# rotationalio/honu

Measured on AMD Instinct MI355X. Metric: GiB/s + records/s device-resident encode+decode, 1M Large(~300KB) object batch, higher is better.
Workload: dtype u8

## Files before the change

### honu_amd/csrc/lane.h

```cpp
#pragma once

#include "common.h"

namespace honu {

HONU_DEV void window16(const u32x4 a, const u32x4 b, uint32_t s, uint64_t &lo, uint64_t &hi) {
    const uint32_t q4 = s >> 2, sh = s & 3;
    const uint32_t w0 = a.x, w1 = a.y, w2 = a.z, w3 = a.w, w4 = b.x, w5 = b.y, w6 = b.z, w7 = b.w;
    const bool o1 = q4 & 1, o2 = q4 & 2;
#define PICK(j0, j1, j2, j3) (o2 ? (o1 ? (j3) : (j2)) : (o1 ? (j1) : (j0)))
    const uint32_t p0 = PICK(w0, w1, w2, w3);
    const uint32_t p1 = PICK(w1, w2, w3, w4);
    const uint32_t p2 = PICK(w2, w3, w4, w5);
    const uint32_t p3 = PICK(w3, w4, w5, w6);
    const uint32_t p4 = PICK(w4, w5, w6, w7);
#undef PICK
    const uint32_t r0 = __builtin_amdgcn_alignbyte(p1, p0, sh);
    const uint32_t r1 = __builtin_amdgcn_alignbyte(p2, p1, sh);
    const uint32_t r2 = __builtin_amdgcn_alignbyte(p3, p2, sh);
    const uint32_t r3 = __builtin_amdgcn_alignbyte(p4, p3, sh);
    lo = ((uint64_t)r1 << 32) | r0;
    hi = ((uint64_t)r3 << 32) | r2;
}

HONU_DEV void lane_fetch16(const uint8_t *__restrict__ base, uint64_t q, uint64_t end,
                           uint64_t &lo, uint64_t &hi) {
    const uint64_t A = q & ~15ull;
    const uint32_t s = (uint32_t)(q & 15);
    const u32x4 a = *reinterpret_cast<const u32x4 *>(base + A);
    u32x4 b = {0, 0, 0, 0};
    if (s && A + 16 < end) b = *reinterpret_cast<const u32x4 *>(base + A + 16);
    window16(a, b, s, lo, hi);
}

HONU_DEV uint64_t compact7(uint64_t x) {
    x = (x & 0x007F007F007F007Full) | ((x & 0x7F007F007F007F00ull) >> 1);
    x = (x & 0x00003FFF00003FFFull) | ((x & 0x3FFF00003FFF0000ull) >> 2);
    x = (x & 0x000000000FFFFFFFull) | ((x & 0x0FFFFFFF00000000ull) >> 4);
    return x;
}

HONU_DEV uint32_t uvarint_window(uint64_t lo, uint64_t hi, uint32_t n, uint64_t &v) {
    const uint64_t tl = ~lo & 0x8080808080808080ull;
    const uint64_t th = ~hi & 0x0000000000008080ull;
    uint32_t k;
    if (tl) k = (uint32_t)(__builtin_ctzll(tl) >> 3) + 1;
    else if (th) k = (uint32_t)(__builtin_ctzll(th) >> 3) + 9;
    else k = 11;
    if (k > n) return 0;
    if (k == 10 && ((hi >> 8) & 0xFF) > 1) return 0;
    const uint64_t m = k >= 8 ? lo : (lo & ((1ull << (8 * k)) - 1));
    uint64_t x = compact7(m & 0x7F7F7F7F7F7F7F7Full);
    if (k >= 9) x |= (hi & 0x7F) << 56;
    if (k == 10) x |= ((hi >> 8) & 0x7F) << 63;
    v = x;
    return k;
}

template <int NDW> struct RowT {
    uint32_t d[NDW];
    HONU_DEV void clear() {
#pragma unroll
        for (int i = 0; i < NDW; i++) d[i] = 0;
    }
    HONU_DEV void u8(int off, uint32_t v) { d[off >> 2] |= (v & 0xFF) << (8 * (off & 3)); }
    HONU_DEV void u32(int off, uint32_t v) { d[off >> 2] = v; }
    HONU_DEV void u64(int off, uint64_t v) {
        d[off >> 2] = (uint32_t)v;
        d[(off >> 2) + 1] = (uint32_t)(v >> 32);
    }
    HONU_DEV void bytes16(int off, uint64_t lo, uint64_t hi) {
        u64(off, lo);
        u64(off + 8, hi);
    }
    HONU_DEV void span(int off, uint64_t o, uint64_t l) {
        u64(off, o);
        u64(off + 8, l);
    }
    template <class T> HONU_DEV void store(T *dst) const {
        static_assert(sizeof(T) == 4 * NDW, "row size");
        u32x4 *p = reinterpret_cast<u32x4 *>(dst);
#pragma unroll
        for (int i = 0; i < NDW / 4; i++)
            p[i] = u32x4{d[4 * i], d[4 * i + 1], d[4 * i + 2], d[4 * i + 3]};
    }
};
using Row = RowT<88>;

struct GlobalSrc {
    const uint8_t *base;
    HONU_DEV uint32_t u8(uint64_t p) const { return base[p]; }
    HONU_DEV void fetch16(uint64_t p, uint64_t end, uint64_t &lo, uint64_t &hi) const {
        lane_fetch16(base, p, end, lo, hi);
    }
};

template <class Src> struct DecT {
    Src src;
    uint64_t p, end, tstart;

    HONU_DEV int u8(uint32_t &v) {
        if (p >= end) return HONU_ERR_EOF;
        v = src.u8(p);
        p += 1;
        return HONU_OK;
    }
    HONU_DEV int boolean(uint32_t &v) {
        int st = u8(v);
        if (st) return st;
        return v > 1 ? HONU_ERR_PARSE_BOOLEAN : HONU_OK;
    }
    HONU_DEV int uv(uint32_t maxw, int err, uint64_t &v) {
        if (p >= end) return HONU_ERR_EOF;
        const uint64_t avail = end - p;
        const uint32_t n = avail < maxw ? (uint32_t)avail : maxw;
        uint64_t lo, hi;
        src.fetch16(p, end, lo, hi);
        const uint32_t k = uvarint_window(lo, hi, n, v);
        if (!k) return err;
        p += k;
        return HONU_OK;
    }
    HONU_DEV int u32(uint32_t &v) {
        uint64_t x = 0;
        int st = uv(5, HONU_ERR_PARSE_VARINT, x);
        v = (uint32_t)x;
        return st;
    }
    HONU_DEV int u64(uint64_t &v) { return uv(10, HONU_ERR_PARSE_VARINT, v); }
    HONU_DEV int i64(int64_t &v) {
        uint64_t x = 0;
        int st = uv(10, HONU_ERR_PARSE_VARINT, x);
        v = unzigzag(x);
        return st;
    }
    HONU_DEV int ulid(uint64_t &lo, uint64_t &hi) {
        if (p >= end) return HONU_ERR_EOF;
        if (p + 16 > end) return HONU_ERR_UNEXPECTED_EOF;
        src.fetch16(p, end, lo, hi);
        p += 16;
        return HONU_OK;
    }
    HONU_DEV int frame(uint64_t &off, uint64_t &len) {
        uint64_t rl = 0;
        int st = uv(10, HONU_ERR_NO_LENGTH, rl);
        if (st) return st;
        if (rl >= (1ull << 63)) return HONU_ERR_PANIC;
        if (rl == 0) {
            off = 0;
            len = 0;
            return HONU_OK;
        }
        if (rl > (uint64_t)INT64_MAX - (p - tstart)) return HONU_ERR_PANIC;
        if (p + rl > end) return HONU_ERR_UNEXPECTED_EOF;
        off = p;
        len = rl;
        p += rl;
        return HONU_OK;
    }
};
using LaneDec = DecT<GlobalSrc>;

HONU_DEV uint32_t uvarint_bytes(uint64_t x, uint64_t &lo, uint64_t &hi) {
    const uint32_t n = uvarint_len(x);
    uint64_t y = x & 0x00FFFFFFFFFFFFFFull;
    y = (y & 0x000000000FFFFFFFull) | ((y & 0x00FFFFFFF0000000ull) << 4);
    y = (y & 0x00003FFF00003FFFull) | ((y & 0x0FFFC0000FFFC000ull) << 2);
    y = (y & 0x007F007F007F007Full) | ((y & 0x3F803F803F803F80ull) << 1);
    const uint32_t nl = n < 8 ? n : 8;
    const uint64_t cont = n > 8 ? 0x8080808080808080ull
                                : (0x8080808080808080ull & ((1ull << (8 * (nl - 1))) - 1));
    lo = (y | cont) & (nl == 8 ? ~0ull : ((1ull << (8 * nl)) - 1));
    hi = 0;
    if (n > 8) hi = ((x >> 56) & 0x7F) | (n > 9 ? 0x80 : 0) | ((x >> 63) << 8);
    return n;
}

template <int R>
struct LaneWriterT {
    uint8_t *out;
    uint64_t cpos;
    uint32_t f;
    uint32_t first;
    uint64_t a0, a1;
    uint64_t hpos;
    uint32_t hfirst;
    uint64_t h0, h1;
    u32x4 *ring;
    uint32_t nch;

    HONU_DEV void init(uint8_t *o, uint64_t pos) {
        out = o;
        cpos = pos & ~15ull;
        f = first = (uint32_t)(pos & 15);
        a0 = a1 = 0;
        hfirst = 0;
        nch = 0;
    }
    HONU_DEV void set_ring(u32x4 *r) { ring = r; }
    static HONU_DEV void store_bytes(uint8_t *p, uint32_t from, uint32_t to, uint64_t b0, uint64_t b1) {
        uint32_t j = from;
        auto bytes_at = [&](uint32_t k, uint32_t n) -> uint64_t {
            uint64_t v = k < 8 ? (b0 >> (8 * k)) | (k ? b1 << (64 - 8 * k) : 0) : b1 >> (8 * (k - 8));
            return n == 8 ? v : v & ((1ull << (8 * n)) - 1);
        };
        if ((j & 1) && j < to) { p[j] = (uint8_t)bytes_at(j, 1); j += 1; }
        if ((j & 2) && j + 2 <= to) { *reinterpret_cast<uint16_t *>(p + j) = (uint16_t)bytes_at(j, 2); j += 2; }
        if ((j & 4) && j + 4 <= to) { *reinterpret_cast<uint32_t *>(p + j) = (uint32_t)bytes_at(j, 4); j += 4; }
        if (j + 8 <= to) { *reinterpret_cast<uint64_t *>(p + j) = bytes_at(j, 8); j += 8; }
        if (j + 4 <= to) { *reinterpret_cast<uint32_t *>(p + j) = (uint32_t)bytes_at(j, 4); j += 4; }
        if (j + 2 <= to) { *reinterpret_cast<uint16_t *>(p + j) = (uint16_t)bytes_at(j, 2); j += 2; }
        if (j < to) p[j] = (uint8_t)bytes_at(j, 1);
    }
    HONU_DEV void flush() {
        if (first == 0) {
            const u32x4 v{(uint32_t)a0, (uint32_t)(a0 >> 32), (uint32_t)a1, (uint32_t)(a1 >> 32)};
            if constexpr (R > 0) {
                ring[((cpos >> 4) & (R - 1)) * HONU_WAVE] = v;
                nch++;
            } else {
                *reinterpret_cast<u32x4 *>(out + cpos) = v;
            }
        } else {
            hpos = cpos;
            hfirst = first;
            h0 = a0;
            h1 = a1;
            first = 0;
        }
        cpos += 16;
    }
    HONU_DEV void put(uint64_t v, uint32_t n) {
        const uint32_t s = 8 * f;
        uint64_t t2 = 0;
        if (s < 64) {
            a0 |= v << s;
            if (s) a1 |= v >> (64 - s);
        } else {
            a1 |= v << (s - 64);
            if (s > 64) t2 = v >> (128 - s);
        }
        f += n;
        if (f >= 16) {
            flush();
            a0 = t2;
            a1 = 0;
            f -= 16;
        }
    }
    HONU_DEV void byte(uint32_t v) { put(v & 0xFF, 1); }
    HONU_DEV void put16(uint64_t lo, uint64_t hi) {
        put(lo, 8);
        put(hi, 8);
    }
    HONU_DEV void uv(uint64_t x) {
        uint64_t lo, hi;
        const uint32_t n = uvarint_bytes(x, lo, hi);
        put(lo, n < 8 ? n : 8);
        if (n > 8) put(hi, n - 8);
    }
    HONU_DEV void run(const uint8_t *src, uint64_t len) {
        const uint64_t a = (uint64_t)src & 15;
        const u32x4 *w = reinterpret_cast<const u32x4 *>(src - a);
        const uint64_t nw = (a + len + 15) >> 4;
        const uint32_t sh = (uint32_t)(a & 7) * 8, hw = (uint32_t)(a >> 3);
        for (uint64_t k = 0; k < len; k += 64) {
            drain();
            const uint64_t q0 = (a + k) >> 4;
            uint64_t x[11];
#pragma unroll
            for (int j = 0; j < 5; j++) {
                u32x4 v{0, 0, 0, 0};
                if (q0 + j < nw) v = w[q0 + j];
                x[2 * j] = ((uint64_t)v.y << 32) | v.x;
                x[2 * j + 1] = ((uint64_t)v.w << 32) | v.z;
            }
            x[10] = 0;
#pragma unroll
            for (int j = 0; j < 8; j++) {
                const uint64_t off = k + 8 * j;
                if (off < len) {
                    const uint64_t take = len - off < 8 ? len - off : 8;
                    const uint64_t lo = hw ? x[j + 1] : x[j], hi = hw ? x[j + 2] : x[j + 1];
                    uint64_t v = sh ? (lo >> sh) | (hi << (64 - sh)) : lo;
                    if (take < 8) v &= (1ull << (8 * take)) - 1;
                    put(v, (uint32_t)take);
                }
            }
        }
    }
    HONU_DEV void frame(const uint8_t *var, honu_span sp) {
        uv(sp.len);
        run(var + sp.off, sp.len);
    }
    HONU_DEV void drain_all() {
        if constexpr (R > 0) {
            const uint64_t p0 = cpos - 16ull * nch;
            for (uint32_t k = 0; k < nch; k++)
                *reinterpret_cast<u32x4 *>(out + p0 + 16 * k) = ring[(((p0 >> 4) + k) & (R - 1)) * HONU_WAVE];
            nch = 0;
        }
    }
    HONU_DEV void drain() {
        if constexpr (R == 16) {
            const uint64_t p0 = cpos - 16ull * nch, lim = cpos & ~127ull;
            if (p0 < lim) {
                const uint32_t cnt = (uint32_t)((lim - p0) >> 4);
                for (uint32_t k = 0; k < cnt; k++)
                    *reinterpret_cast<u32x4 *>(out + p0 + 16 * k) = ring[(((p0 >> 4) + k) & (R - 1)) * HONU_WAVE];
                nch -= cnt;
            }
        } else {
            drain_all();
        }
    }
    HONU_DEV void finish() {
        drain_all();
        if (hfirst) store_bytes(out + hpos, hfirst, 16, h0, h1);
        hfirst = 0;
        if (f > first) store_bytes(out + cpos, first, f, a0, a1);
    }
    HONU_DEV uint64_t pos() const { return cpos + f; }
    HONU_DEV void jump(uint64_t to) {
        finish();
        cpos = to & ~15ull;
        f = first = (uint32_t)(to & 15);
        a0 = a1 = 0;
    }
};
using LaneWriter = LaneWriterT<0>;


#ifdef HONU_ENC_TIMING
#define ENC_STAMPS 8
static __device__ uint64_t g_enc_stamps[1 << 16][ENC_STAMPS];
#define ESTAMP(k)                                                                             \
    do {                                                                                      \
        const uint64_t wid_ = (uint64_t)blockIdx.x * (blockDim.x / 64) + threadIdx.x / 64;    \
        if (__lane_id() == 0 && wid_ < (1 << 16)) g_enc_stamps[wid_][k] = wall_clock64();     \
    } while (0)
#else
#define ESTAMP(k) \
    do {          \
    } while (0)
#endif

HONU_DEV uint64_t ld64(const uint8_t *p) { return *reinterpret_cast<const uint64_t *>(p); }

#ifndef ACL_UNIT
#define ACL_UNIT 16ull
#endif
#ifndef HONU_ACL_ENDS
#define HONU_ACL_ENDS 0
#endif
template <bool SKIP_ACL, int R>
HONU_DEV uint64_t encode_record_lane(const honu_meta &m, const uint8_t *__restrict__ var,
                                     const honu_acl *__restrict__ acl,
                                     const uint32_t *__restrict__ reg, uint64_t dlen,
                                     uint64_t beg, uint64_t end, uint8_t *__restrict__ out,
                                     u32x4 *ring, const uint8_t *__restrict__ psrc = nullptr) {
    static_assert(R == 0 || ((R == 8 || R == 16) && SKIP_ACL),
                  "drain spacing assumes 8 slots (16 with line drains: <= 7 held + <= 7 new) and no ACL entries");
#define OFF(f) ((int)offsetof(honu_meta, f))
    uint64_t acl_ret = 0;
    ESTAMP(1);
    const uint8_t *mb = reinterpret_cast<const uint8_t *>(&m);
    const uint32_t pr = m.present;
    LaneWriterT<R> W;
    W.set_ring(ring);
    if (psrc) {
        W.init(out, beg);
        W.byte(HONU_STORAGE_VERSION);
        W.uv(dlen);
        const uint64_t a0 = (uint64_t)out + W.pos(), a1 = a0 + dlen;
        const uint64_t h_end = ((a0 + PAYLOAD_UNIT - 1) & ~(PAYLOAD_UNIT - 1)) < a1
                                   ? ((a0 + PAYLOAD_UNIT - 1) & ~(PAYLOAD_UNIT - 1)) : a1;
        const uint64_t t_beg = (a1 & ~(PAYLOAD_UNIT - 1)) > h_end ? (a1 & ~(PAYLOAD_UNIT - 1)) : h_end;
        W.run(psrc, h_end - a0);
        if (t_beg > h_end) W.jump(t_beg - (uint64_t)out);
        W.run(psrc + (t_beg - a0), a1 - t_beg);
        W.drain();
    } else {
        uint64_t lo, hi;
        const uint32_t hn = uvarint_bytes(dlen, lo, hi);
        out[beg] = HONU_STORAGE_VERSION;
        for (uint32_t j = 0; j < hn; j++)
            out[beg + 1 + j] = (uint8_t)(j < 8 ? lo >> (8 * j) : hi >> (8 * (j - 8)));
        W.init(out, beg + 1 + uvarint_len(dlen) + dlen);
    }
    W.byte(1);
    W.put16(ld64(mb + OFF(object_id)), ld64(mb + OFF(object_id) + 8));
    W.put16(ld64(mb + OFF(collection_id)), ld64(mb + OFF(collection_id) + 8));
    if (pr & HONU_HAS_VERSION) {
        W.byte(1);
        W.uv(m.pid);
        W.uv(m.vid);
        W.uv(m.region);
        if (pr & HONU_HAS_PARENT) {
            W.byte(1);
            W.uv(m.parent_pid);
            W.uv(m.parent_vid);
        } else {
            W.byte(0);
        }
        W.byte(m.tombstone ? 1 : 0);
        W.uv(zigzag(m.version_created));
    } else {
        W.byte(0);
    }
    W.drain();
    if (pr & HONU_HAS_SCHEMA) {
        W.byte(1);
        W.frame(var, m.schema_name);
        W.uv(m.schema_major);
        W.uv(m.schema_minor);
        W.uv(m.schema_patch);
    } else {
        W.byte(0);
    }
    W.drain();
    W.frame(var, m.mime);
    W.drain();
    ESTAMP(2);
    W.put16(ld64(mb + OFF(owner)), ld64(mb + OFF(owner) + 8));
    W.put16(ld64(mb + OFF(group)), ld64(mb + OFF(group) + 8));
    W.byte(m.permissions);
    const uint64_t na = m.acl_count, ao = m.acl_off;
    W.uv(na);
    const uint64_t nr = m.regions_count, ro = m.regions_off;
    ESTAMP(3);
    if constexpr (SKIP_ACL) {
        const uint64_t P = W.pos();
        uint64_t sfx = uvarint_len(nr) + 3 + 1 + uvarint_len(zigzag(m.created)) +
                       uvarint_len(zigzag(m.modified));
        for (uint64_t k0 = 0; k0 < nr; k0 += 8) {
            uint32_t r8[8];
#pragma unroll
            for (int j = 0; j < 8; j++) r8[j] = k0 + j < nr ? reg[ro + k0 + j] : 0;
#pragma unroll
            for (int j = 0; j < 8; j++) sfx += k0 + j < nr ? uvarint_len(r8[j]) : 0;
        }
        if (pr & HONU_HAS_PUBLISHER) sfx += 32 + frame_len(m.ip_address.len) + frame_len(m.user_agent.len);
        if (pr & HONU_HAS_ENCRYPTION)
            sfx += frame_len(m.public_key_id.len) + frame_len(m.encryption_key.len) +
                   frame_len(m.hmac_secret.len) + frame_len(m.signature.len) + 3;
        if (pr & HONU_HAS_COMPRESSION) sfx += 1 + uvarint_len(zigzag(m.compression_level));
        const uint64_t E = end - sfx;
        if (na && E - P == 18 * na) {
            acl_ret = P | ACL_ALL_PRESENT;
            const uint64_t ab = (uint64_t)out;
            const uint64_t hu = ((ab + P + ACL_UNIT - 1) & ~(ACL_UNIT - 1)) - ab;
            const uint64_t hend = hu < E ? hu : E;
            const uint64_t tu = ((ab + E) & ~(ACL_UNIT - 1)) - ab;
            const uint64_t T = tu > hend ? tu : hend;
            auto put_n = [&](const u32x4 &v, uint32_t cnt) {
                const uint64_t lo = ((uint64_t)v.y << 32) | v.x, hi = ((uint64_t)v.w << 32) | v.z;
                if (cnt >= 8) {
                    W.put(lo, 8);
                    if (cnt == 16) W.put(hi, 8);
                    else if (cnt > 8) W.put(hi & ((1ull << (8 * (cnt - 8))) - 1), cnt - 8);
                } else if (cnt) {
                    W.put(lo & ((1ull << (8 * cnt)) - 1), cnt);
                }
            };
            if constexpr (HONU_ACL_ENDS && ACL_UNIT == 16) {
                W.jump(E);
            } else if constexpr (ACL_UNIT == 16) {
                const u32x4 hv = acl_chunk(acl + ao, na, P, P);
                const u32x4 tv = E > T ? acl_chunk(acl + ao, na, P, T) : u32x4{0, 0, 0, 0};
                put_n(hv, (uint32_t)(hend - P));
                if (T > hend) W.jump(T);
                put_n(tv, (uint32_t)(E - T));
            } else {
                W.drain();
                for (uint64_t x = P; x < hend; x += 16)
                    put_n(acl_chunk(acl + ao, na, P, x), (uint32_t)(hend - x < 16 ? hend - x : 16));
                if (T > hend) W.jump(T);
                for (uint64_t x = T; x < E; x += 16)
                    put_n(acl_chunk(acl + ao, na, P, x), (uint32_t)(E - x < 16 ? E - x : 16));
                W.drain();
            }
        } else {
            acl_ret = P;
            W.jump(E);
        }
    } else {
    for (uint64_t k0 = 0; k0 < na; k0 += 8) {
        uint32_t e[8][5];
#pragma unroll
        for (int j = 0; j < 8; j++) {
            if (k0 + j < na) {
                const uint32_t *a = reinterpret_cast<const uint32_t *>(acl + ao + k0 + j);
#pragma unroll
                for (int c = 0; c < 5; c++) e[j][c] = a[c];
            }
        }
#pragma unroll
        for (int j = 0; j < 8; j++) {
            if (k0 + j < na) {
                if ((e[j][4] >> 8) & 0xFF) {
                    W.byte(1);
                    W.put16(((uint64_t)e[j][1] << 32) | e[j][0], ((uint64_t)e[j][3] << 32) | e[j][2]);
                    W.byte(e[j][4]);
                } else {
                    W.byte(0);
                }
            }
        }
    }
    }
    ESTAMP(4);
    W.uv(nr);
    for (uint64_t k0 = 0; k0 < nr; k0 += 8) {
        uint32_t r8[8];
#pragma unroll
        for (int j = 0; j < 8; j++) r8[j] = k0 + j < nr ? reg[ro + k0 + j] : 0;
        W.drain();
#pragma unroll
        for (int j = 0; j < 8; j++)
            if (k0 + j < nr) W.uv(r8[j]);
    }
    W.drain();
    ESTAMP(5);
    if (pr & HONU_HAS_PUBLISHER) {
        W.byte(1);
        W.put16(ld64(mb + OFF(publisher_id)), ld64(mb + OFF(publisher_id) + 8));
        W.put16(ld64(mb + OFF(client_id)), ld64(mb + OFF(client_id) + 8));
        W.frame(var, m.ip_address);
        W.frame(var, m.user_agent);
    } else {
        W.byte(0);
    }
    W.drain();
    ESTAMP(6);
    if (pr & HONU_HAS_ENCRYPTION) {
        W.byte(1);
        W.frame(var, m.public_key_id);
        W.frame(var, m.encryption_key);
        W.frame(var, m.hmac_secret);
        W.frame(var, m.signature);
        W.byte(m.sealing_alg);
        W.byte(m.encryption_alg);
        W.byte(m.signature_alg);
    } else {
        W.byte(0);
    }
    W.drain();
    if (pr & HONU_HAS_COMPRESSION) {
        W.byte(1);
        W.byte(m.compression_alg);
        W.uv(zigzag(m.compression_level));
    } else {
        W.byte(0);
    }
    W.byte(m.flags);
    W.uv(zigzag(m.created));
    W.uv(zigzag(m.modified));
    W.finish();
    ESTAMP(7);
    return acl_ret;
}
#undef OFF

}
```

Before: 1176.

## Prefetch variable-length fields into registers before emitting them in lane encoder

Adds a GatherT register buffer that loads aligned 16-byte words of each variable-length field (payload head/tail, schema, mime, ip, user agent, key ids, hmac, signature) well before they are written. Region values and ACL head/tail chunks are also loaded early, so the global loads are issued up front and overlap instead of each one stalling right when its field is emitted. This raises register pressure, since many u32x4 blocks are live at once, which may lower occupancy. Fields longer than the gather coverage fall back to the old run path.

Result: no change. 1184 (median of 2 runs) (+0.7%).

```diff
diff --git a/honu_amd/csrc/lane.h b/honu_amd/csrc/lane.h
--- a/honu_amd/csrc/lane.h
+++ b/honu_amd/csrc/lane.h
@@ -176,6 +176,21 @@
     return n;
 }
 
+template <int B> struct GatherT {
+    static constexpr uint32_t COVER = 16 * B - 16;
+    u32x4 v[B];
+    HONU_DEV void load(const uint8_t *src, uint64_t len) {
+        const uint64_t a = (uint64_t)src & 15;
+        const u32x4 *w = reinterpret_cast<const u32x4 *>(src - a);
+        const uint64_t nw = len ? (a + len + 15) >> 4 : 0;
+#pragma unroll
+        for (int j = 0; j < B; j++) {
+            v[j] = u32x4{0, 0, 0, 0};
+            if ((uint64_t)j < nw) v[j] = w[j];
+        }
+    }
+};
+
 template <int R>
 struct LaneWriterT {
     uint8_t *out;
@@ -293,6 +308,35 @@
         uv(sp.len);
         run(var + sp.off, sp.len);
     }
+    template <bool REST = true, int B>
+    HONU_DEV void emit(const GatherT<B> &g, const uint8_t *src, uint64_t len) {
+        const uint32_t a = (uint32_t)((uint64_t)src & 15);
+        const uint32_t sh = (a & 7) * 8, hw = a >> 3;
+        uint64_t x[2 * B];
+#pragma unroll
+        for (int j = 0; j < B; j++) {
+            x[2 * j] = ((uint64_t)g.v[j].y << 32) | g.v[j].x;
+            x[2 * j + 1] = ((uint64_t)g.v[j].w << 32) | g.v[j].z;
+        }
+#pragma unroll
+        for (int j = 0; j < 2 * B - 2; j++) {
+            const uint64_t off = 8 * j;
+            if (off < len) {
+                if (j % 8 == 0) drain();
+                const uint64_t take = len - off < 8 ? len - off : 8;
+                const uint64_t lo = hw ? x[j + 1] : x[j], hi = hw ? x[j + 2] : x[j + 1];
+                uint64_t v = sh ? (lo >> sh) | (hi << (64 - sh)) : lo;
+                if (take < 8) v &= (1ull << (8 * take)) - 1;
+                put(v, (uint32_t)take);
+            }
+        }
+        if constexpr (REST)
+            if (len > GatherT<B>::COVER) run(src + GatherT<B>::COVER, len - GatherT<B>::COVER);
+    }
+    template <int B> HONU_DEV void frame(const GatherT<B> &g, const uint8_t *var, honu_span sp) {
+        uv(sp.len);
+        emit(g, var + sp.off, sp.len);
+    }
     HONU_DEV void drain_all() {
         if constexpr (R > 0) {
             const uint64_t p0 = cpos - 16ull * nch;
@@ -353,6 +397,7 @@
 #ifndef HONU_ACL_ENDS
 #define HONU_ACL_ENDS 0
 #endif
+constexpr int SIG_BLOCKS = 9;
 template <bool SKIP_ACL, int R>
 HONU_DEV uint64_t encode_record_lane(const honu_meta &m, const uint8_t *__restrict__ var,
                                      const honu_acl *__restrict__ acl,
@@ -366,19 +411,30 @@
     ESTAMP(1);
     const uint8_t *mb = reinterpret_cast<const uint8_t *>(&m);
     const uint32_t pr = m.present;
+    const bool has_sch = pr & HONU_HAS_SCHEMA, has_pub = pr & HONU_HAS_PUBLISHER;
+    const bool has_enc = pr & HONU_HAS_ENCRYPTION;
+    const uint64_t nr = m.regions_count, ro = m.regions_off;
     LaneWriterT<R> W;
     W.set_ring(ring);
+    const uint64_t a0 = (uint64_t)out + beg + 1 + uvarint_len(dlen), a1 = a0 + dlen;
+    const uint64_t h_end = ((a0 + PAYLOAD_UNIT - 1) & ~(PAYLOAD_UNIT - 1)) < a1
+                               ? ((a0 + PAYLOAD_UNIT - 1) & ~(PAYLOAD_UNIT - 1)) : a1;
+    const uint64_t t_beg = (a1 & ~(PAYLOAD_UNIT - 1)) > h_end ? (a1 & ~(PAYLOAD_UNIT - 1)) : h_end;
+    GatherT<5> g_head, g_tail;
+    GatherT<3> g_schema, g_mime;
+    if (psrc) {
+        g_head.load(psrc, h_end - a0);
+        g_tail.load(psrc + (t_beg - a0), a1 - t_beg);
+    }
+    g_schema.load(var + m.schema_name.off, has_sch ? m.schema_name.len : 0);
+    g_mime.load(var + m.mime.off, m.mime.len);
     if (psrc) {
         W.init(out, beg);
         W.byte(HONU_STORAGE_VERSION);
         W.uv(dlen);
-        const uint64_t a0 = (uint64_t)out + W.pos(), a1 = a0 + dlen;
-        const uint64_t h_end = ((a0 + PAYLOAD_UNIT - 1) & ~(PAYLOAD_UNIT - 1)) < a1
-                                   ? ((a0 + PAYLOAD_UNIT - 1) & ~(PAYLOAD_UNIT - 1)) : a1;
-        const uint64_t t_beg = (a1 & ~(PAYLOAD_UNIT - 1)) > h_end ? (a1 & ~(PAYLOAD_UNIT - 1)) : h_end;
-        W.run(psrc, h_end - a0);
+        W.template emit<false>(g_head, psrc, h_end - a0);
         if (t_beg > h_end) W.jump(t_beg - (uint64_t)out);
-        W.run(psrc + (t_beg - a0), a1 - t_beg);
+        W.template emit<false>(g_tail, psrc + (t_beg - a0), a1 - t_beg);
         W.drain();
     } else {
         uint64_t lo, hi;
@@ -388,6 +444,15 @@
             out[beg + 1 + j] = (uint8_t)(j < 8 ? lo >> (8 * j) : hi >> (8 * (j - 8)));
         W.init(out, beg + 1 + uvarint_len(dlen) + dlen);
     }
+    uint32_t r8[8];
+#pragma unroll
+    for (int j = 0; j < 8; j++) r8[j] = (uint64_t)j < nr ? reg[ro + j] : 0;
+    GatherT<2> g_ip;
+    GatherT<3> g_ua, g_pkid, g_ekey;
+    g_ip.load(var + m.ip_address.off, has_pub ? m.ip_address.len : 0);
+    g_ua.load(var + m.user_agent.off, has_pub ? m.user_agent.len : 0);
+    g_pkid.load(var + m.public_key_id.off, has_enc ? m.public_key_id.len : 0);
+    g_ekey.load(var + m.encryption_key.off, has_enc ? m.encryption_key.len : 0);
     W.byte(1);
     W.put16(ld64(mb + OFF(object_id)), ld64(mb + OFF(object_id) + 8));
     W.put16(ld64(mb + OFF(collection_id)), ld64(mb + OFF(collection_id) + 8));
@@ -409,9 +474,9 @@
         W.byte(0);
     }
     W.drain();
-    if (pr & HONU_HAS_SCHEMA) {
+    if (has_sch) {
         W.byte(1);
-        W.frame(var, m.schema_name);
+        W.frame(g_schema, var, m.schema_name);
         W.uv(m.schema_major);
         W.uv(m.schema_minor);
         W.uv(m.schema_patch);
@@ -419,7 +484,7 @@
         W.byte(0);
     }
     W.drain();
-    W.frame(var, m.mime);
+    W.frame(g_mime, var, m.mime);
     W.drain();
     ESTAMP(2);
     W.put16(ld64(mb + OFF(owner)), ld64(mb + OFF(owner) + 8));
@@ -427,32 +492,41 @@
     W.byte(m.permissions);
     const uint64_t na = m.acl_count, ao = m.acl_off;
     W.uv(na);
-    const uint64_t nr = m.regions_count, ro = m.regions_off;
     ESTAMP(3);
     if constexpr (SKIP_ACL) {
         const uint64_t P = W.pos();
         uint64_t sfx = uvarint_len(nr) + 3 + 1 + uvarint_len(zigzag(m.created)) +
                        uvarint_len(zigzag(m.modified));
-        for (uint64_t k0 = 0; k0 < nr; k0 += 8) {
-            uint32_t r8[8];
-#pragma unroll
-            for (int j = 0; j < 8; j++) r8[j] = k0 + j < nr ? reg[ro + k0 + j] : 0;
-#pragma unroll
-            for (int j = 0; j < 8; j++) sfx += k0 + j < nr ? uvarint_len(r8[j]) : 0;
-        }
-        if (pr & HONU_HAS_PUBLISHER) sfx += 32 + frame_len(m.ip_address.len) + frame_len(m.user_agent.len);
-        if (pr & HONU_HAS_ENCRYPTION)
+#pragma unroll
+        for (int j = 0; j < 8; j++) sfx += (uint64_t)j < nr ? uvarint_len(r8[j]) : 0;
+        for (uint64_t k0 = 8; k0 < nr; k0 += 8) {
+            uint32_t q8[8];
+#pragma unroll
+            for (int j = 0; j < 8; j++) q8[j] = k0 + j < nr ? reg[ro + k0 + j] : 0;
+#pragma unroll
+            for (int j = 0; j < 8; j++) sfx += k0 + j < nr ? uvarint_len(q8[j]) : 0;
+        }
+        if (has_pub) sfx += 32 + frame_len(m.ip_address.len) + frame_len(m.user_agent.len);
+        if (has_enc)
             sfx += frame_len(m.public_key_id.len) + frame_len(m.encryption_key.len) +
                    frame_len(m.hmac_secret.len) + frame_len(m.signature.len) + 3;
         if (pr & HONU_HAS_COMPRESSION) sfx += 1 + uvarint_len(zigzag(m.compression_level));
         const uint64_t E = end - sfx;
-        if (na && E - P == 18 * na) {
+        const bool all_present = na && E - P == 18 * na;
+        const uint64_t ab = (uint64_t)out;
+        const uint64_t hu = ((ab + P + ACL_UNIT - 1) & ~(ACL_UNIT - 1)) - ab;
+        const uint64_t hend = hu < E ? hu : E;
+        const uint64_t tu = ((ab + E) & ~(ACL_UNIT - 1)) - ab;
+        const uint64_t T = tu > hend ? tu : hend;
+        u32x4 hv{0, 0, 0, 0}, tv{0, 0, 0, 0};
+        if constexpr (!HONU_ACL_ENDS && ACL_UNIT == 16) {
+            if (all_present) {
+                hv = acl_chunk(acl + ao, na, P, P);
+                if (E > T) tv = acl_chunk(acl + ao, na, P, T);
+            }
+        }
+        if (all_present) {
             acl_ret = P | ACL_ALL_PRESENT;
-            const uint64_t ab = (uint64_t)out;
-            const uint64_t hu = ((ab + P + ACL_UNIT - 1) & ~(ACL_UNIT - 1)) - ab;
-            const uint64_t hend = hu < E ? hu : E;
-            const uint64_t tu = ((ab + E) & ~(ACL_UNIT - 1)) - ab;
-            const uint64_t T = tu > hend ? tu : hend;
             auto put_n = [&](const u32x4 &v, uint32_t cnt) {
                 const uint64_t lo = ((uint64_t)v.y << 32) | v.x, hi = ((uint64_t)v.w << 32) | v.z;
                 if (cnt >= 8) {
@@ -466,8 +540,6 @@
             if constexpr (HONU_ACL_ENDS && ACL_UNIT == 16) {
                 W.jump(E);
             } else if constexpr (ACL_UNIT == 16) {
-                const u32x4 hv = acl_chunk(acl + ao, na, P, P);
-                const u32x4 tv = E > T ? acl_chunk(acl + ao, na, P, T) : u32x4{0, 0, 0, 0};
                 put_n(hv, (uint32_t)(hend - P));
                 if (T > hend) W.jump(T);
                 put_n(tv, (uint32_t)(E - T));
@@ -511,34 +583,47 @@
     }
     ESTAMP(4);
     W.uv(nr);
-    for (uint64_t k0 = 0; k0 < nr; k0 += 8) {
-        uint32_t r8[8];
-#pragma unroll
-        for (int j = 0; j < 8; j++) r8[j] = k0 + j < nr ? reg[ro + k0 + j] : 0;
+    if (nr) W.drain();
+#pragma unroll
+    for (int j = 0; j < 8; j++)
+        if ((uint64_t)j < nr) W.uv(r8[j]);
+    for (uint64_t k0 = 8; k0 < nr; k0 += 8) {
+        uint32_t q8[8];
+#pragma unroll
+        for (int j = 0; j < 8; j++) q8[j] = k0 + j < nr ? reg[ro + k0 + j] : 0;
         W.drain();
 #pragma unroll
         for (int j = 0; j < 8; j++)
-            if (k0 + j < nr) W.uv(r8[j]);
+            if (k0 + j < nr) W.uv(q8[j]);
     }
     W.drain();
     ESTAMP(5);
-    if (pr & HONU_HAS_PUBLISHER) {
+    GatherT<3> g_hmac;
+    GatherT<SIG_BLOCKS> g_sig, g_sig2;
+    const uint8_t *sig = var + m.signature.off;
+    const uint64_t sig1 = !has_enc ? 0 : m.signature.len < g_sig.COVER ? m.signature.len : g_sig.COVER;
+    g_hmac.load(var + m.hmac_secret.off, has_enc ? m.hmac_secret.len : 0);
+    g_sig.load(sig, sig1);
+    if (has_pub) {
         W.byte(1);
         W.put16(ld64(mb + OFF(publisher_id)), ld64(mb + OFF(publisher_id) + 8));
         W.put16(ld64(mb + OFF(client_id)), ld64(mb + OFF(client_id) + 8));
-        W.frame(var, m.ip_address);
-        W.frame(var, m.user_agent);
+        W.frame(g_ip, var, m.ip_address);
+        W.frame(g_ua, var, m.user_agent);
     } else {
         W.byte(0);
     }
     W.drain();
     ESTAMP(6);
-    if (pr & HONU_HAS_ENCRYPTION) {
+    g_sig2.load(sig + g_sig.COVER, has_enc ? m.signature.len - sig1 : 0);
+    if (has_enc) {
         W.byte(1);
-        W.frame(var, m.public_key_id);
-        W.frame(var, m.encryption_key);
-        W.frame(var, m.hmac_secret);
-        W.frame(var, m.signature);
+        W.frame(g_pkid, var, m.public_key_id);
+        W.frame(g_ekey, var, m.encryption_key);
+        W.frame(g_hmac, var, m.hmac_secret);
+        W.uv(m.signature.len);
+        W.template emit<false>(g_sig, sig, sig1);
+        W.emit(g_sig2, sig + g_sig.COVER, m.signature.len - sig1);
         W.byte(m.sealing_alg);
         W.byte(m.encryption_alg);
         W.byte(m.signature_alg);
```
